# bottledspace/refraction-raytracing-dxr

Measured on AMD Instinct MI355X. Metric: Mrays/s (primary+refracted) at 1920x1080, monkey.obj, higher is better.
Workload: dtype f32

## Files before the change

### refraction_raytracing_dxr_amd/csrc/rr_launch.h

```cpp
#pragma once
#include <hip/hip_runtime.h>
#include "rr_types.h"
#include "host/rr_host_lens.h"

namespace rr {

struct alignas(16) rr_ray_dev { float origin[3]; float tmin; float dir[3]; float tmax; uint32_t flags; uint32_t instance_mask; uint32_t pad[2]; };
struct rr_hit_dev { float t, u, v; uint32_t prim, inst, hit; };
static_assert(sizeof(rr_ray_dev) == 48 && sizeof(rr_hit_dev) == 24, "ABI layout");

hipError_t launch_render_fused(const SceneDev& sc, const DispatchDev& a, int stack, int pend, bool stats, hipStream_t s,
                               bool stack16 = false);
const char* last_render_kernel_name();
void set_render_kernel_name(const char* fmt, ...) __attribute__((format(printf, 1, 2)));
hipError_t launch_render_paths(const SceneDev& sc, const DispatchDev& a, int stack, bool stats, hipStream_t s);
int lds_kernel_shape(uint32_t node_bytes, uint32_t stack_entries, size_t* lds_bytes, int min_shape = 0);
hipError_t launch_render_lds(const SceneDev& sc, const DispatchDev& a, LdsDispatch q, int n_cus, bool stats, hipStream_t s, int min_shape = 0);
hipError_t launch_render_stream(const SceneDev& sc, const DispatchDev& a, const StreamDev& s, int stack, uint32_t n_wg, bool stats, hipStream_t st);
hipError_t launch_env_lookup(const SceneDev& sc, const float* dirs, uint32_t n, float* rgb, hipStream_t s);
hipError_t launch_trace_rays(const SceneDev& sc, const rr_ray_dev* rays, uint32_t n, rr_hit_dev* hits, uint32_t* err,
                             int stack, hipStream_t s);
hipError_t launch_query_rays(const SceneDev& sc, const rr_ray_dev* rays, uint32_t n, rr_hit_dev* hits, uint32_t inst0_mask, int stack,
                             hipStream_t s);
constexpr uint32_t RR_QUERY_MULTI_MAX_K = 16;
hipError_t launch_query_multi(const SceneDev& sc, const rr_ray_dev* rays, uint32_t n, uint32_t k, rr_hit_dev* hits, uint32_t* counts,
                              uint32_t inst0_mask, int stack, hipStream_t s);
hipError_t launch_shade_rays(const SceneDev& sc, const DispatchDev& a, const rr_ray_dev* rays, uint32_t n, float4* f32, uint32_t* rgba8,
                             uint32_t* n_rays, int stack, int pend, bool stack16, hipStream_t s);
struct SampleOffsets { static constexpr uint32_t MAX = 64; float v[2 * MAX]; };
hipError_t launch_render_samples(const SceneDev& sc, const DispatchDev& a, const CamDev& cam, const SampleOffsets& off, uint32_t n_samples,
                                 float4* f32, uint32_t* rgba8, uint32_t* n_rays, int stack, int pend, bool stack16, hipStream_t s);
hipError_t launch_render_lens(const SceneDev& sc, const DispatchDev& a, const CamDev& cam, const SampleOffsets& off, const SampleOffsets& loff,
                              const LensDev& lens, uint32_t n_samples, float4* f32, uint32_t* rgba8, uint32_t* n_rays, int stack, int pend,
                              bool stack16, hipStream_t s);
struct BandTable { static constexpr uint32_t MAX = SampleOffsets::MAX; float ior[MAX]; float inv_ior[MAX]; float weight[MAX][3]; };
hipError_t launch_render_spectral(const SceneDev& sc, const DispatchDev& a, const CamDev& cam, const SampleOffsets& off, const BandTable& bands,
                                  uint32_t n_samples, float4* f32, uint32_t* rgba8, uint32_t* n_rays, int stack, int pend, bool stack16,
                                  hipStream_t s);
hipError_t launch_shade_rays_mat(const SceneDev& sc, const DispatchDev& a, const MatDev* mats, uint32_t mat0, const rr_ray_dev* rays, uint32_t n,
                                 float4* f32, uint32_t* rgba8, uint32_t* n_rays, int stack, int pend, bool stack16, hipStream_t s);
hipError_t launch_render_materials(const SceneDev& sc, const DispatchDev& a, const CamDev& cam, const SampleOffsets& off, const MatDev* mats,
                                   uint32_t mat0, uint32_t n_samples, float4* f32, uint32_t* rgba8, uint32_t* n_rays, int stack, int pend,
                                   bool stack16, hipStream_t s);
struct AdaptiveWorkspace {
    float4* rec; uint32_t* cnt; uint32_t* list; unsigned long long* masks; uint32_t* base; uint32_t* total;
    uint64_t bytes;
    AdaptiveWorkspace(void* p, uint32_t W, uint32_t H)
    {
        const uint64_t n = (uint64_t)W * H, nb = (uint64_t)((W + 7u) / 8u) * ((H + 7u) / 8u);
        const uint64_t o_cnt = 16u * n, o_list = o_cnt + 4u * n, o_masks = (o_list + 4u * n + 15u) & ~(uint64_t)15u, o_base = o_masks + 8u * nb;
        const uintptr_t c = reinterpret_cast<uintptr_t>(p);
        rec = static_cast<float4*>(p); cnt = reinterpret_cast<uint32_t*>(c + o_cnt); list = reinterpret_cast<uint32_t*>(c + o_list);
        masks = reinterpret_cast<unsigned long long*>(c + o_masks); base = reinterpret_cast<uint32_t*>(c + o_base); total = base + nb;
        bytes = (o_base + 4u * (nb + 1u) + 15u) & ~(uint64_t)15u;
    }
};
hipError_t launch_render_adaptive(const SceneDev& sc, const DispatchDev& a, const CamDev& cam, const SampleOffsets& off, uint32_t n_base,
                                  uint32_t n_max, float threshold, const AdaptiveWorkspace& ws, float4* f32, uint32_t* rgba8, uint32_t* n_rays,
                                  uint32_t* n_taken, int stack, int pend, bool stack16, uint32_t refine_groups, hipStream_t s);
hipError_t launch_screen_tables(float* out, uint32_t W, uint32_t H, hipStream_t s);
hipError_t launch_assemble_tiles(const uint32_t* gathered, uint32_t* frame, uint32_t W, uint32_t H, uint32_t tiles_x,
                                 uint32_t n_tiles, uint32_t world, uint32_t max_tiles, hipStream_t s);
hipError_t launch_assemble_frames(const uint32_t* gathered, uint32_t* frames, uint32_t W, uint32_t H, uint32_t tiles_x,
                                  uint32_t n_tiles, uint32_t world, size_t rank_stride, size_t frame_stride,
                                  size_t out_stride, uint32_t n_frames, hipStream_t s);
hipError_t launch_assemble_frames_rgb8(const uint8_t* gathered, uint32_t* frames, uint32_t W, uint32_t H, uint32_t tiles_x, uint32_t n_tiles,
                                       uint32_t world, size_t rank_stride_b, size_t frame_stride_b, size_t out_stride, uint32_t n_frames,
                                       hipStream_t s);
hipError_t launch_assemble_frames_mesh_rgb8(const uint8_t* gathered, const uint8_t* bg, uint32_t* frames, uint32_t W, uint32_t H, const MeshPartDev& mp,
                                            size_t rank_stride_b, size_t frame_stride_b, size_t bg_stride_b, size_t out_stride, uint32_t n_frames, hipStream_t s);

struct BuildBuffers {
    uint32_t n;
    uint32_t n_pad;
    float*   prim_box;
    unsigned long long* keys;
    int32_t* parent;
    int32_t* child;
    float*   node_box;
    uint32_t* visit;
    uint32_t* scene_box;
    uint32_t* depth;
    uint32_t* ploc;
    BvhNode* nodes;
    uint32_t leaf_ref_prim;
    uint32_t leaf_base;
};

hipError_t launch_tri_setup(const void* verts, const uint32_t* idx, uint32_t n_tris, const BuildBuffers& b, hipStream_t s);
hipError_t launch_lbvh(const BuildBuffers& b, hipStream_t s);
constexpr uint32_t PLOC_MAX_PRIMS = 32768;
hipError_t launch_ploc(const BuildBuffers& b, hipStream_t s);
hipError_t launch_pack_tris(const void* verts, const uint32_t* idx, const BuildBuffers& b, TriRec* tris, NrmRec* nrms,
                            hipStream_t s);
hipError_t launch_inst_setup(const InstDev* insts, const float* blas_bounds, uint32_t n, const BuildBuffers& b, hipStream_t s);
hipError_t launch_quantize_nodes(QNode* dst, const BvhNode* src, uint32_t n_nodes, const QGrid& g, uint32_t node_off, uint32_t tri_off,
                                 hipStream_t s);
hipError_t launch_keep_links(const BuildBuffers& b, int32_t* links, hipStream_t s);
hipError_t launch_refit_blas(const void* verts, const uint32_t* idx, uint32_t n_tris, TriRec* tris, NrmRec* nrms, BvhNode* nodes,
                             const int32_t* links, uint32_t* visit, uint32_t* scene_box, hipStream_t s);
hipError_t launch_refit_tlas(const InstDev* insts, const float* xforms_and_bounds, uint32_t n, BvhNode* nodes, const int32_t* links,
                             uint32_t* visit, hipStream_t s);
hipError_t launch_update_verts(const void* d_src, void* d_dst, uint32_t n_verts, uint32_t* st, hipStream_t s);
hipError_t launch_env_pad(const float* rgb, float4* out, uint32_t n_texels, hipStream_t s);

}
```

### refraction_raytracing_dxr_amd/csrc/rr_render_fused.hip

```cpp
#include <hip/hip_runtime.h>
#include <cstdarg>
#include <cstdio>
#include "rr_render_common.h"

namespace rr {

template <int STACK, int PEND, bool STATS, bool TLAS, bool DIAG = false, class E = uint32_t, int WPS = 0>
__global__ __launch_bounds__(256, WPS ? WPS : TLAS ? RR_TLAS_WAVES_PER_SIMD(STACK) : sizeof(E) == 2 ? 8 : RR_FUSED_WAVES_PER_SIMD(STACK)) void k_render_fused(SceneDev sc, DispatchDev a)
{
    __shared__ uint32_t diag_trips[12];
    const unsigned long long diag_t0 = DIAG ? __builtin_amdgcn_s_memtime() : 0ull;
    const unsigned long long diag_rt0 = DIAG ? __builtin_amdgcn_s_memrealtime() : 0ull;
    if (DIAG && threadIdx.x < 12) diag_trips[threadIdx.x] = 0;
    if (DIAG) __syncthreads();
    extern __shared__ __attribute__((aligned(16))) uint32_t lds[];
    const uint32_t wave = __builtin_amdgcn_readfirstlane(threadIdx.x >> 6), lane = threadIdx.x & 63u;
    E* stk = reinterpret_cast<E*>(lds) + wave * (STACK * 64) + lane;

    const BlockPos bp = wave_block_pos(a, blockIdx.x * 4u + wave);
    const uint32_t lx = compact1by1(lane), ly = compact1by1(lane >> 1);
    const uint32_t x = bp.x0 + lx, y = bp.y0 + ly;
    const bool valid = bp.tile_ok && x < a.W && y < a.H;
    const CamDev& cb = a.cams[bp.frame];

    LaneStats st;
    stats_clock_begin<STATS>(st);
    st.blocks = bp.tile_ok ? 1u : 0u;
    if (STATS && bp.tile_ok && !(DIAG || (bp.x0 + 8u > a.hx0 && bp.x0 < a.hx1 && bp.y0 + 8u > a.hy0 && bp.y0 < a.hy1))) st.bg_blocks = 1u;
    if (valid) {
        st.pixels = 1;
        const bool may_hit = DIAG || (bp.x0 + 8u > a.hx0 && bp.x0 < a.hx1 && bp.y0 + 8u > a.hy0 && bp.y0 < a.hy1);
        f3 acc;
        if (!may_hit) {
            const f3 D = camera_ray_dir(cb.M, a.sx[x], a.sy[y]);
            st.rays = 1;
            if (STATS) { st.miss = 1; if (first_active_lane()) st.passes = 1; }
            const f3 e = env_lookup(sc, D);
            acc = mk3(fmaf(1.0f, e.x, 0.0f), fmaf(1.0f, e.y, 0.0f), fmaf(1.0f, e.z, 0.0f));
        } else {
            RegPark<PEND> park;
            acc = render_pixel<STATS, TLAS, DIAG, E, GlobalNodes>(sc, a, cb, x, y, true, stk, GlobalNodes{}, park, st, Diag{ &diag_trips[wave], 4 });
        }
        typedef const __attribute__((address_space(4))) DispatchDev* KA;
        KA ap = (KA)((const __attribute__((address_space(4))) char*)__builtin_amdgcn_kernarg_segment_ptr() +
                     ((sizeof(SceneDev) + alignof(DispatchDev) - 1) / alignof(DispatchDev)) * alignof(DispatchDev));
        asm volatile("" : "+s"(ap));
        const uint32_t k_compact = ap->compact_out, k_W = ap->W, k_tonemap = ap->tonemap;
        const size_t o = k_compact == 0u ? (size_t)y * k_W + x
                                         : (size_t)bp.tile_local * (TILE * TILE) + (bp.py0 + ly) * TILE + (bp.px0 + lx);
        uint32_t* const out_rgba8 = bp.bg ? ap->out_bg + (size_t)bp.frame * ap->bg_stride : ap->out_rgba8 + (size_t)bp.frame * ap->frame_stride;
        float4* const out_f32 = ap->out_f32 ? ap->out_f32 + (size_t)bp.frame * ap->frame_stride : nullptr;
        DispatchDev a2;
        a2.tonemap = k_tonemap; a2.compact_out = k_compact;
        store_pixel(a2, out_rgba8, out_f32, o, acc);
    }

    if (DIAG) {
        uint32_t mx = st.rays;
        for (int off = 32; off > 0; off >>= 1) { uint32_t v = __shfl_xor(mx, off, 64); mx = v > mx ? v : mx; }
        if (lane == 0) {
            unsigned long long* d = a.diag + (size_t)(blockIdx.x * 4u + wave) * 4;
            d[0] = ((unsigned long long)diag_trips[8 + wave] << 40) | ((unsigned long long)diag_trips[4 + wave] << 20) | diag_trips[wave];
            d[1] = __builtin_amdgcn_s_memtime() - diag_t0; d[2] = mx | ((diag_rt0 & 0xffffffffull) << 32);
            d[3] = (unsigned long long)(diag_trips[wave] + diag_trips[4 + wave]) | ((__builtin_amdgcn_s_memrealtime() & 0xffffffffull) << 32);
        }
    }
    flush_stats<STATS>(a, st, blockIdx.x * 4u + wave, lane);
}

static thread_local char g_kernel_name[96] = "";
const char* last_render_kernel_name() { return g_kernel_name; }
void set_render_kernel_name(const char* fmt, ...)
{
    va_list ap;
    va_start(ap, fmt);
    vsnprintf(g_kernel_name, sizeof g_kernel_name, fmt, ap);
    va_end(ap);
}

template <int STACK, int PEND, bool TLAS>
static hipError_t launch_fused_spt(const SceneDev& sc, const DispatchDev& a, bool stats, hipStream_t s)
{
    const size_t lds = (size_t)4 * STACK * 64 * sizeof(uint32_t);
    set_render_kernel_name("k_render_fused<%d, %d, %s, %s, false, unsigned int, 0>", STACK, PEND, stats ? "true" : "false", TLAS ? "true" : "false");
    if (stats) hipLaunchKernelGGL((k_render_fused<STACK, PEND, true, TLAS>), dim3(a.n_blocks), dim3(256), lds, s, sc, a);
    else       hipLaunchKernelGGL((k_render_fused<STACK, PEND, false, TLAS>), dim3(a.n_blocks), dim3(256), lds, s, sc, a);
    return hipGetLastError();
}

template <int STACK, int PEND>
static hipError_t launch_fused_sp(const SceneDev& sc, const DispatchDev& a, bool stats, hipStream_t s)
{
    if (!sc.single_identity) return launch_fused_spt<STACK, PEND, true>(sc, a, stats, s);
    return launch_fused_spt<STACK, PEND, false>(sc, a, stats, s);
}

template <int PEND>
static hipError_t launch_fused_s16(const SceneDev& sc, const DispatchDev& a, bool stats, hipStream_t s)
{
    const size_t lds = (size_t)4 * 39 * 64 * sizeof(uint16_t);
    set_render_kernel_name("k_render_fused<39, %d, %s, false, false, unsigned short, 0>", PEND, stats ? "true" : "false");
    if (stats) hipLaunchKernelGGL((k_render_fused<39, PEND, true, false, false, uint16_t>), dim3(a.n_blocks), dim3(256), lds, s, sc, a);
    else       hipLaunchKernelGGL((k_render_fused<39, PEND, false, false, false, uint16_t>), dim3(a.n_blocks), dim3(256), lds, s, sc, a);
    return hipGetLastError();
}

template <int STACK, int WPS>
static hipError_t launch_fused_tlas16(const SceneDev& sc, const DispatchDev& a, bool stats, hipStream_t s)
{
    const size_t lds = (size_t)4 * STACK * 64 * sizeof(uint16_t);
    set_render_kernel_name("k_render_fused<%d, 2, %s, true, false, unsigned short, %d>", STACK, stats ? "true" : "false", WPS);
    if (stats) hipLaunchKernelGGL((k_render_fused<STACK, 2, true, true, false, uint16_t, WPS>), dim3(a.n_blocks), dim3(256), lds, s, sc, a);
    else       hipLaunchKernelGGL((k_render_fused<STACK, 2, false, true, false, uint16_t, WPS>), dim3(a.n_blocks), dim3(256), lds, s, sc, a);
    return hipGetLastError();
}

hipError_t launch_render_fused(const SceneDev& sc, const DispatchDev& a, int stack, int pend, bool stats, hipStream_t s, bool stack16)
{
    if (a.n_blocks == 0) return hipSuccess;
#ifndef RR_TLAS30_WPS
#define RR_TLAS30_WPS 7
#endif
#ifndef RR_TLAS39_WPS
#define RR_TLAS39_WPS 5
#endif
    if (stack16 && !a.diag && !sc.single_identity && pend <= 2 && stack <= 30) return launch_fused_tlas16<30, RR_TLAS30_WPS>(sc, a, stats, s);
    if (stack16 && !a.diag && !sc.single_identity && pend <= 2 && stack <= 39) return launch_fused_tlas16<39, RR_TLAS39_WPS>(sc, a, stats, s);
    if (stack16 && !a.diag && sc.single_identity && stack <= 39)
        return pend <= 2 ? launch_fused_s16<2>(sc, a, stats, s) : launch_fused_s16<8>(sc, a, stats, s);
    if (a.diag) {
        if (stack <= 19) hipLaunchKernelGGL((k_render_fused<19, 2, false, false, true>), dim3(a.n_blocks), dim3(256), 4 * 19 * 64 * 4, s, sc, a);
        else hipLaunchKernelGGL((k_render_fused<31, 2, false, false, true>), dim3(a.n_blocks), dim3(256), 4 * 31 * 64 * 4, s, sc, a);
        return hipGetLastError();
    }
    if (stack <= 19 && pend <= 2) return launch_fused_sp<19, 2>(sc, a, stats, s);
    if (stack <= 22 && pend <= 2) return launch_fused_sp<22, 2>(sc, a, stats, s);
    if (stack <= 26 && pend <= 2) return launch_fused_sp<26, 2>(sc, a, stats, s);
    if (stack <= 31) return pend <= 2 ? launch_fused_sp<31, 2>(sc, a, stats, s) : launch_fused_sp<31, 8>(sc, a, stats, s);
    if (stack <= 39) return pend <= 2 ? launch_fused_sp<39, 2>(sc, a, stats, s) : launch_fused_sp<39, 8>(sc, a, stats, s);
    return pend <= 2 ? launch_fused_sp<64, 2>(sc, a, stats, s) : launch_fused_sp<64, 8>(sc, a, stats, s);
}

}
```

Baseline: 31770.

## Size fused render workgroups to the smallest wave count that fills LDS occupancy

The fused render kernel's workgroup size is no longer fixed at four waves. It now picks 1, 2 or 4 waves per group using a compile-time model of LDS allocation granules and per-CU wave limits. Each group's waves are mapped back to the same 32x8 strips through an XCD-aware block index. This aims to cut LDS fragmentation and the per-group co-scheduling limits that cap resident waves, in exchange for more and smaller blocks and a new block-to-tile mapping that may change cache locality across XCDs.

```diff
diff --git a/refraction_raytracing_dxr_amd/csrc/rr_launch.h b/refraction_raytracing_dxr_amd/csrc/rr_launch.h
--- a/refraction_raytracing_dxr_amd/csrc/rr_launch.h
+++ b/refraction_raytracing_dxr_amd/csrc/rr_launch.h
@@ -9,6 +9,31 @@
 struct rr_hit_dev { float t, u, v; uint32_t prim, inst, hit; };
 static_assert(sizeof(rr_ray_dev) == 48 && sizeof(rr_hit_dev) == 24, "ABI layout");
 
+#ifndef RR_FUSED_GROUP_WAVES
+#define RR_FUSED_GROUP_WAVES 0
+#endif
+constexpr uint32_t LDS_GRANULE = 1280u, LDS_GRANULES_PER_CU = 128u, WAVES_PER_CU = 32u;
+constexpr uint32_t resident_waves_per_cu(uint32_t g, uint32_t bytes_per_wave)
+{
+    const uint32_t granules = (g * bytes_per_wave + LDS_GRANULE - 1u) / LDS_GRANULE;
+    const uint32_t groups = granules == 0u || LDS_GRANULES_PER_CU / granules > WAVES_PER_CU / g ? WAVES_PER_CU / g : LDS_GRANULES_PER_CU / granules;
+    return groups * g;
+}
+constexpr uint32_t fused_group_waves(uint32_t stack, uint32_t entry_bytes, uint32_t waves_per_simd)
+{
+    if (RR_FUSED_GROUP_WAVES) return RR_FUSED_GROUP_WAVES;
+    for (uint32_t g = 1u; g < 4u; g *= 2u)
+        if (resident_waves_per_cu(g, stack * 64u * entry_bytes) >= 4u * waves_per_simd) return g;
+    return 4u;
+}
+static_assert(RR_FUSED_GROUP_WAVES == 0 || RR_FUSED_GROUP_WAVES == 1 || RR_FUSED_GROUP_WAVES == 2 || RR_FUSED_GROUP_WAVES == 4, "a 32x8 strip is four wave-blocks");
+__host__ __device__ constexpr uint32_t fused_wave_block(uint32_t b, uint32_t g)
+{
+    const uint32_t per_strip = 4u / g;
+    const uint32_t xcd = b & 7u, j = b >> 3;
+    const uint32_t blk = (j / per_strip) * 8u + xcd;
+    return blk * 4u + (j % per_strip) * g;
+}
 hipError_t launch_render_fused(const SceneDev& sc, const DispatchDev& a, int stack, int pend, bool stats, hipStream_t s,
                                bool stack16 = false);
 const char* last_render_kernel_name();
diff --git a/refraction_raytracing_dxr_amd/csrc/rr_render_fused.hip b/refraction_raytracing_dxr_amd/csrc/rr_render_fused.hip
--- a/refraction_raytracing_dxr_amd/csrc/rr_render_fused.hip
+++ b/refraction_raytracing_dxr_amd/csrc/rr_render_fused.hip
@@ -5,19 +5,29 @@
 
 namespace rr {
 
+template <int STACK, bool TLAS, class E, int WPS> struct FusedShape {
+    static constexpr int waves_per_simd = WPS ? WPS : TLAS ? RR_TLAS_WAVES_PER_SIMD(STACK) : sizeof(E) == 2 ? 8 : RR_FUSED_WAVES_PER_SIMD(STACK);
+    static constexpr uint32_t group_waves = fused_group_waves(STACK, sizeof(E), waves_per_simd);
+    static constexpr uint32_t threads = 64u * group_waves;
+    static constexpr size_t lds_bytes = (size_t)group_waves * STACK * 64 * sizeof(E);
+    static dim3 grid(const DispatchDev& a) { return dim3(a.n_blocks * (4u / group_waves)); }
+};
+
 template <int STACK, int PEND, bool STATS, bool TLAS, bool DIAG = false, class E = uint32_t, int WPS = 0>
-__global__ __launch_bounds__(256, WPS ? WPS : TLAS ? RR_TLAS_WAVES_PER_SIMD(STACK) : sizeof(E) == 2 ? 8 : RR_FUSED_WAVES_PER_SIMD(STACK)) void k_render_fused(SceneDev sc, DispatchDev a)
+__global__ __launch_bounds__((FusedShape<STACK, TLAS, E, WPS>::threads), (FusedShape<STACK, TLAS, E, WPS>::waves_per_simd)) void k_render_fused(SceneDev sc, DispatchDev a)
 {
+    constexpr uint32_t GW = FusedShape<STACK, TLAS, E, WPS>::group_waves;
     __shared__ uint32_t diag_trips[12];
     const unsigned long long diag_t0 = DIAG ? __builtin_amdgcn_s_memtime() : 0ull;
     const unsigned long long diag_rt0 = DIAG ? __builtin_amdgcn_s_memrealtime() : 0ull;
     if (DIAG && threadIdx.x < 12) diag_trips[threadIdx.x] = 0;
     if (DIAG) __syncthreads();
     extern __shared__ __attribute__((aligned(16))) uint32_t lds[];
-    const uint32_t wave = __builtin_amdgcn_readfirstlane(threadIdx.x >> 6), lane = threadIdx.x & 63u;
+    const uint32_t wave = GW == 1u ? 0u : __builtin_amdgcn_readfirstlane(threadIdx.x >> 6), lane = threadIdx.x & 63u;
     E* stk = reinterpret_cast<E*>(lds) + wave * (STACK * 64) + lane;
 
-    const BlockPos bp = wave_block_pos(a, blockIdx.x * 4u + wave);
+    const uint32_t wb = fused_wave_block(blockIdx.x, GW) + wave;
+    const BlockPos bp = wave_block_pos(a, wb);
     const uint32_t lx = compact1by1(lane), ly = compact1by1(lane >> 1);
     const uint32_t x = bp.x0 + lx, y = bp.y0 + ly;
     const bool valid = bp.tile_ok && x < a.W && y < a.H;
@@ -59,13 +69,13 @@
         uint32_t mx = st.rays;
         for (int off = 32; off > 0; off >>= 1) { uint32_t v = __shfl_xor(mx, off, 64); mx = v > mx ? v : mx; }
         if (lane == 0) {
-            unsigned long long* d = a.diag + (size_t)(blockIdx.x * 4u + wave) * 4;
+            unsigned long long* d = a.diag + (size_t)wb * 4;
             d[0] = ((unsigned long long)diag_trips[8 + wave] << 40) | ((unsigned long long)diag_trips[4 + wave] << 20) | diag_trips[wave];
             d[1] = __builtin_amdgcn_s_memtime() - diag_t0; d[2] = mx | ((diag_rt0 & 0xffffffffull) << 32);
             d[3] = (unsigned long long)(diag_trips[wave] + diag_trips[4 + wave]) | ((__builtin_amdgcn_s_memrealtime() & 0xffffffffull) << 32);
         }
     }
-    flush_stats<STATS>(a, st, blockIdx.x * 4u + wave, lane);
+    flush_stats<STATS>(a, st, wb, lane);
 }
 
 static thread_local char g_kernel_name[96] = "";
@@ -78,13 +88,19 @@
     va_end(ap);
 }
 
+template <int STACK, int PEND, bool STATS, bool TLAS, bool DIAG = false, class E = uint32_t, int WPS = 0>
+static void launch_fused(const SceneDev& sc, const DispatchDev& a, hipStream_t s)
+{
+    using Shape = FusedShape<STACK, TLAS, E, WPS>;
+    hipLaunchKernelGGL((k_render_fused<STACK, PEND, STATS, TLAS, DIAG, E, WPS>), Shape::grid(a), dim3(Shape::threads), Shape::lds_bytes, s, sc, a);
+}
+
 template <int STACK, int PEND, bool TLAS>
 static hipError_t launch_fused_spt(const SceneDev& sc, const DispatchDev& a, bool stats, hipStream_t s)
 {
-    const size_t lds = (size_t)4 * STACK * 64 * sizeof(uint32_t);
     set_render_kernel_name("k_render_fused<%d, %d, %s, %s, false, unsigned int, 0>", STACK, PEND, stats ? "true" : "false", TLAS ? "true" : "false");
-    if (stats) hipLaunchKernelGGL((k_render_fused<STACK, PEND, true, TLAS>), dim3(a.n_blocks), dim3(256), lds, s, sc, a);
-    else       hipLaunchKernelGGL((k_render_fused<STACK, PEND, false, TLAS>), dim3(a.n_blocks), dim3(256), lds, s, sc, a);
+    if (stats) launch_fused<STACK, PEND, true, TLAS>(sc, a, s);
+    else       launch_fused<STACK, PEND, false, TLAS>(sc, a, s);
     return hipGetLastError();
 }
 
@@ -98,20 +114,18 @@
 template <int PEND>
 static hipError_t launch_fused_s16(const SceneDev& sc, const DispatchDev& a, bool stats, hipStream_t s)
 {
-    const size_t lds = (size_t)4 * 39 * 64 * sizeof(uint16_t);
     set_render_kernel_name("k_render_fused<39, %d, %s, false, false, unsigned short, 0>", PEND, stats ? "true" : "false");
-    if (stats) hipLaunchKernelGGL((k_render_fused<39, PEND, true, false, false, uint16_t>), dim3(a.n_blocks), dim3(256), lds, s, sc, a);
-    else       hipLaunchKernelGGL((k_render_fused<39, PEND, false, false, false, uint16_t>), dim3(a.n_blocks), dim3(256), lds, s, sc, a);
+    if (stats) launch_fused<39, PEND, true, false, false, uint16_t>(sc, a, s);
+    else       launch_fused<39, PEND, false, false, false, uint16_t>(sc, a, s);
     return hipGetLastError();
 }
 
 template <int STACK, int WPS>
 static hipError_t launch_fused_tlas16(const SceneDev& sc, const DispatchDev& a, bool stats, hipStream_t s)
 {
-    const size_t lds = (size_t)4 * STACK * 64 * sizeof(uint16_t);
     set_render_kernel_name("k_render_fused<%d, 2, %s, true, false, unsigned short, %d>", STACK, stats ? "true" : "false", WPS);
-    if (stats) hipLaunchKernelGGL((k_render_fused<STACK, 2, true, true, false, uint16_t, WPS>), dim3(a.n_blocks), dim3(256), lds, s, sc, a);
-    else       hipLaunchKernelGGL((k_render_fused<STACK, 2, false, true, false, uint16_t, WPS>), dim3(a.n_blocks), dim3(256), lds, s, sc, a);
+    if (stats) launch_fused<STACK, 2, true, true, false, uint16_t, WPS>(sc, a, s);
+    else       launch_fused<STACK, 2, false, true, false, uint16_t, WPS>(sc, a, s);
     return hipGetLastError();
 }
 
@@ -129,8 +143,8 @@
     if (stack16 && !a.diag && sc.single_identity && stack <= 39)
         return pend <= 2 ? launch_fused_s16<2>(sc, a, stats, s) : launch_fused_s16<8>(sc, a, stats, s);
     if (a.diag) {
-        if (stack <= 19) hipLaunchKernelGGL((k_render_fused<19, 2, false, false, true>), dim3(a.n_blocks), dim3(256), 4 * 19 * 64 * 4, s, sc, a);
-        else hipLaunchKernelGGL((k_render_fused<31, 2, false, false, true>), dim3(a.n_blocks), dim3(256), 4 * 31 * 64 * 4, s, sc, a);
+        if (stack <= 19) launch_fused<19, 2, false, false, true>(sc, a, s);
+        else launch_fused<31, 2, false, false, true>(sc, a, s);
         return hipGetLastError();
     }
     if (stack <= 19 && pend <= 2) return launch_fused_sp<19, 2>(sc, a, stats, s);
```

New measurement: 34520, median of 6. 1.09x the previous value.
